# Diamondfan/CTC_pytorch

Measured on AMD Instinct MI355X. Metric: acoustic frames/sec/GPU (train) + utterances/sec beam-decode (`decode` object), TIMIT 4x320 BiLSTM, higher is better.
Workload: dtype f32 via bf16x3 split-operand MFMA (f32 accumulate); 1 GPU; cfg2: 4x320 BiLSTM + BN + Linear(62) + CTC, B=32/GPU, T=800, F=40, dropout 0.1, Adam; global_batch=32, seq_len=800, parallelism=dp1, full_length_utterances=True, sync_bn=False

## Files before the change

ctc_pytorch_amd/_lib.py:

```python
import ctypes
import glob
import os
import subprocess

import torch

_HERE = os.path.dirname(os.path.abspath(__file__))
_CSRC = os.path.join(_HERE, "csrc")
SO_PATH = os.environ.get("CTCN_LIBCTCN") or os.path.join(_HERE, "libctcn.so")
_lib = None

c_void_p, c_int, c_float, c_double, c_size_t, c_u64 = (ctypes.c_void_p, ctypes.c_int, ctypes.c_float,
                                                      ctypes.c_double, ctypes.c_size_t, ctypes.c_uint64)

P, I, F, D, Z, U = c_void_p, c_int, c_float, c_double, c_size_t, c_u64
_SIGS = {
    "ctcn_version": (I, []),
    "ctcn_last_error": (ctypes.c_char_p, []),
    "ctcn_device_cus": (I, []),
    "ctcn_device_xcds": (I, []),
    "ctcn_set_option": (I, [ctypes.c_char_p, I]),
    "ctcn_get_option": (I, [ctypes.c_char_p]),
    "ctcn_option_name": (ctypes.c_char_p, [I]),
    "ctcn_set_status_buffer": (I, [P]),
# ... 23 lines not shown
    "ctcn_bn_bwd_dropout": (I, [P, P, P, P, P, P, P, P, P, I, I, I, I, F, P, Z, P, F, U, U]),
    "ctcn_dropout": (I, [P, P, Z, F, U, U, P]),
    "ctcn_bn_masked_ws_bytes": (Z, [I, I, I]),
    "ctcn_mask_frames": (I, [P, P, P, I, I, I, I, I, P]),
    "ctcn_bn_fwd_train_masked": (I, [P, P, P, P, P, P, P, P, P, I, I, I, I, I, F, F, I, P, Z, P, P]),
    "ctcn_bn_fwd_eval_masked": (I, [P, P, P, P, P, P, P, I, I, I, I, I, F, I, P]),
    "ctcn_bn_bwd_masked": (I, [P, P, P, P, P, P, P, P, P, P, I, I, I, I, I, I, F, P, Z, P]),
    "ctcn_conv2d_ws_bytes": (Z, [I] * 11),
    "ctcn_conv2d_fwd": (I, [P, P, P, P] + [I] * 11 + [P]),
    "ctcn_conv2d_bwd": (I, [P, P, P, P, P, P] + [I] * 11 + [F, P, Z, P]),
    "ctcn_bctf_to_tbcf": (I, [P, P, I, I, I, I, P]),
    "ctcn_tbcf_to_bctf": (I, [P, P, I, I, I, I, P]),
    "ctcn_log_softmax_fwd": (I, [P, P, P, I, I, P]),
    "ctcn_log_softmax_bwd": (I, [P, P, P, I, I, P]),
    "ctcn_argmax": (I, [P, P, I, I, P]),
    "ctcn_rnn_fwd_ex": (I, [I, I, I, I, I, I, P, P, P, P, P, P, P, P, I, P, Z, P, P]),
    "ctcn_rnn_bwd_ex": (I, [I, I, I, I, I, I, P, P, P, P, P, P, P, P, P, P, P, P, P, P, F, I, P, P, Z, P, P]),
    "ctcn_ctc_fwd": (I, [P, P, P, P, P, P, I, I, I, I, P]),
    "ctcn_ctc_bwd": (I, [P, P, P, P, P, P, P, P, I, I, I, I, P]),
    "ctcn_ctc_fwd_both": (I, [P, P, P, P, P, P, P, I, I, I, I, P]),
    "ctcn_ctc_grad": (I, [P, P, P, P, P, P, P, P, P, I, I, I, I, P]),
    "ctcn_sum_f32": (I, [P, P, I, P]),
    "ctcn_ctc_fwd_ex": (I, [P, P, P, P, P, P, P, I, I, I, I, I, P]),
    "ctcn_ctc_grad_ex": (I, [P, P, P, P, P, P, P, P, I, I, I, I, P, I, I, I, I, P]),
    "ctcn_ctc_reduce": (I, [P, P, P, I, I, I, P]),
    "ctcn_ctc_pack_targets": (I, [P, ctypes.c_int64, P, P, I, I, P]),
    "ctcn_ctc_align_ws_bytes": (Z, [I, I, I]),
    "ctcn_ctc_align": (I, [P, P, P, P, P, P, P, P, P, P, I, I, I, I, I, P, Z, P]),
    "ctcn_adam_step": (I, [P, P, P, P, Z, F, F, F, F, F, I, P]),
    "ctcn_grad_norm_ws_bytes": (Z, [Z, I]),
# ... 237 lines not shown
```

ctc_pytorch_amd/csrc/core.hip:

```cpp
#include "common.h"

static thread_local char g_err[512] = "";

void ctcn_set_error(const char *fmt, ...) {
  va_list ap;
  va_start(ap, fmt);
  vsnprintf(g_err, sizeof(g_err), fmt, ap);
  va_end(ap);
}

extern "C" int ctcn_version(void) { return 100; }
extern "C" const char *ctcn_last_error(void) { return g_err; }
extern "C" int ctcn_device_cus(void) {
  int dev = 0, n = 0;
  if (hipGetDevice(&dev) != hipSuccess) return -1;
  if (hipDeviceGetAttribute(&n, hipDeviceAttributeMultiprocessorCount, dev) != hipSuccess) return -1;
  return n;
}

static int g_opt_rnn_persistent = 1;
static int g_opt_handoff = 1;
static int g_opt_poll_depth = 2;
static int g_opt_recurrence_only = 0;
static int g_opt_bwd_scatter = 1;
// ... 18 lines not shown
static int g_opt_gemm_bf16_single = 0;
static int g_opt_gemm_dx_wide = 1;
static int g_opt_xcd_interleave = 1;
static int g_opt_bn_rows4 = 1;
static int g_opt_tn_splits_force = 0;
static int g_opt_tn_splits_xcd = 1;
static int g_opt_beam_generic_threads = 0;
static int g_opt_beam_bitonic = 1;
static int g_opt_beam_cand_global = 0;
static int g_opt_beam_occ2 = 0;
static int g_opt_beam_fast = 1;
static int g_opt_rnn_slow_items = 0;
static int g_opt_rnn_slow_exchange = 0;
static int g_opt_ctc_lattice_skew = 1;
static int g_opt_ctc_slow_wave = 0;
static int g_opt_xcd_interleave_force = 0;
static int *g_status_dev = nullptr;

struct OptionRow { const char *name; int *var; int (*norm)(int); };
static const OptionRow k_options[] = {
  {"rnn_persistent", &g_opt_rnn_persistent, [](int value) -> int { return value; }},
  {"handoff", &g_opt_handoff, [](int value) -> int { return value; }},
  {"poll_depth", &g_opt_poll_depth, [](int value) -> int { return value; }},
  {"rnn_recurrence_only", &g_opt_recurrence_only, [](int value) -> int { return value ? 1 : 0; }},
  {"bwd_scatter", &g_opt_bwd_scatter, [](int value) -> int { return value ? 1 : 0; }},
  {"handoff_tags", &g_opt_handoff_tags, [](int value) -> int { return value ? 1 : 0; }},
  {"side_split_wgs", &g_opt_side_split_wgs, [](int value) -> int { return value < 1 ? 1 : (value > 16 ? 16 : value); }},
  {"gemm_big_tiles", &g_opt_gemm_big_tiles, [](int value) -> int { return value ? 1 : 0; }},
  {"beam_fast", &g_opt_beam_fast, [](int value) -> int { return value ? 1 : 0; }},
  {"conv_dbg", &g_opt_conv_dbg, [](int value) -> int { return value & 7; }},
// ... 13 lines not shown
  {"bwd_item_gather", &g_opt_bwd_item_gather, [](int value) -> int { return value < 0 ? 0 : (value > 2 ? 2 : value); }},
  {"bwd_poll_delay", &g_opt_bwd_poll_delay, [](int value) -> int { return value < 0 ? -1 : (value > 256 ? 256 : value); }},
  {"conv_mfma", &g_opt_conv_mfma, [](int value) -> int { return value ? 1 : 0; }},
  {"edit_wave", &g_opt_edit_wave, [](int value) -> int { return value ? 1 : 0; }},
  {"gemm_tn", &g_opt_gemm_tn, [](int value) -> int { return value != 0; }},
  {"rnn_fused_dropout", &g_opt_rnn_fused_dropout, [](int value) -> int { return value != 0; }},
  {"tag_poll_delay", &g_opt_tag_poll_delay, [](int value) -> int { return value < 0 ? 0 : (value > 64 ? 64 : value); }},
  {"rnn_fwd_tagged", &g_opt_rnn_fwd_tagged, [](int value) -> int { return value ? 1 : 0; }},
  {"gemm_a_inline", &g_opt_gemm_a_inline, [](int value) -> int { return value ? 1 : 0; }},
  {"gemm_dbg", &g_opt_gemm_dbg, [](int value) -> int { return value; }},
  {"gemm_tile256", &g_opt_gemm_tile256, [](int value) -> int { return value ? 1 : 0; }},
  {"xcd_interleave_force", &g_opt_xcd_interleave_force, [](int value) -> int { return value ? 1 : 0; }},
  {"rnn_slow_exchange", &g_opt_rnn_slow_exchange, [](int value) -> int { return value < 0 ? 0 : (value > 4096 ? 4096 : value); }},
  {"ctc_lattice_skew", &g_opt_ctc_lattice_skew, [](int value) -> int { return value ? 1 : 0; }},
  {"ctc_slow_wave", &g_opt_ctc_slow_wave, [](int value) -> int { return value < 0 ? 0 : (value > 15 ? 15 : value); }},
  {"rnn_slow_items", &g_opt_rnn_slow_items, [](int value) -> int { return value < 0 ? 0 : (value > 4096 ? 4096 : value); }},
};
static const int k_noptions = (int)(sizeof(k_options) / sizeof(k_options[0]));
static const OptionRow *find_option(const char *name) {
  if (name)
    for (int i = 0; i < k_noptions; ++i)
      if (!strcmp(name, k_options[i].name)) return &k_options[i];
  return nullptr;
}
extern "C" int ctcn_set_option(const char *name, int value) {
  if (const OptionRow *o = find_option(name)) { *o->var = o->norm(value); return CTCN_OK; }
  ctcn_set_error("ctcn_set_option: unknown option %s", name ? name : "(null)");
  return CTCN_EINVAL;
}
extern "C" int ctcn_get_option(const char *name) {
// ... 15 lines not shown
```

ctc_pytorch_amd/csrc/gemm.hip:

```cpp
#include <algorithm>
#include <type_traits>

#include "common.h"

namespace {

constexpr int BM = 128, BN = 128, BK = 16, PAD = 4;

__device__ __forceinline__ int xcd_band_tile(int bid, int nt) {
  const int xcd = bid & 7, q = nt >> 3, r = nt & 7;
  return (xcd < r ? xcd * (q + 1) : r * (q + 1) + (xcd - r) * q) + (bid >> 3);
}
__device__ __forceinline__ void g2r_kc(const float *__restrict__ src, int ld, int r0, int R, int k0, int Kend,
                                       bool vec, int tid, float (&reg)[8]) {
#pragma unroll
  for (int j = 0; j < 2; ++j) {
    const int idx = tid + 256 * j;
    const int r = idx >> 2, kq = (idx & 3) * 4;
    const int gr = r0 + r, gk = k0 + kq;
    const float *p = src + (size_t)gr * ld + gk;
    if (vec && gr < R && gk + 3 < Kend) {
      const float4 v = *reinterpret_cast<const float4 *>(p);
      reg[4 * j + 0] = v.x; reg[4 * j + 1] = v.y; reg[4 * j + 2] = v.z; reg[4 * j + 3] = v.w;
    } else {
// ... 134 lines not shown
  if (!((xcd_allow >> (x & 15)) & 1u)) return;
  const int nt = tiles_m * tiles_n, total = nt * splits;
  for (;;) {
    if (threadIdx.x == 0) s_item = (int)atomicAdd(queue, 1u);
    __syncthreads();
    const int item = s_item;
    if (item >= total) return;
    f32_tile<TA, TB>(sA, sB, item % nt, item / nt, M, N, K, A, lda, B, ldb, C, ldc, beta, kchunk, ws, tiles_n, vecA, vecB);
    __syncthreads();
  }
}

constexpr int XBK = 32, XLD = 40;
typedef __bf16 bf16x8_t __attribute__((ext_vector_type(8)));

__device__ __forceinline__ void split_bf16(float x, unsigned short &hi, unsigned short &lo) {
  hi = f2bf(x);
  lo = f2bf(x - __uint_as_float((unsigned)hi << 16));
}

__device__ __forceinline__ void x_g2r_kc(const float *__restrict__ src, int ld, int r0, int R, int k0, int Kend, bool vec,
                                         int tid, float (&reg)[16]) {
#pragma unroll
  for (int j = 0; j < 4; ++j) {
    const int idx = tid + 256 * j;
    const int r = idx >> 3, kq = (idx & 7) * 4;
    const int gr = r0 + r, gk = k0 + kq;
    const float *p = src + (size_t)gr * ld + gk;
    if (vec && gr < R && gk + 3 < Kend) {
      const float4 v = *reinterpret_cast<const float4 *>(p);
      reg[4 * j] = v.x; reg[4 * j + 1] = v.y; reg[4 * j + 2] = v.z; reg[4 * j + 3] = v.w;
    } else {
#pragma unroll
      for (int c = 0; c < 4; ++c) reg[4 * j + c] = (gr < R && gk + c < Kend) ? p[c] : 0.0f;
// ... 1753 lines not shown
```

ctc_pytorch_amd/csrc/norm.hip:

```cpp
#include <algorithm>

#include "common.h"

namespace {

struct Pair { double a, b; };

struct StatVal {
  const float *x;
  __device__ __forceinline__ Pair operator()(size_t idx, int) const {
    const double v = x[idx];
    return {v, v * v};
  }
  struct Quad { f32x4 x; };
  __device__ __forceinline__ Quad load4(size_t idx) const { return {*reinterpret_cast<const f32x4 *>(x + idx)}; }
  __device__ __forceinline__ void add4(const Quad &q, int, double &a, double &b) const {
#pragma unroll
    for (int e = 0; e < 4; ++e) { const double v = q.x[e]; a += v; b += v * v; }
  }
  __host__ __device__ __forceinline__ bool aligned16() const { return ((uintptr_t)x & 15) == 0; }
  struct ColK {};
  static constexpr int ROWS_IN_FLIGHT = 8;
  __device__ __forceinline__ ColK colk(int) const { return {}; }
  __device__ __forceinline__ void cols4(const Quad &q, const ColK &, double (&a)[4], double (&b)[4]) const {
#pragma unroll
    for (int e = 0; e < 4; ++e) { const double v = q.x[e]; a[e] += v; b[e] += v * v; }
  }
};
struct DropSpec { float p, scale; uint64_t seed, offset; const float *gamma, *beta; };
__device__ __forceinline__ float bn_value(float x, float m, float rs, float g, float b) { return fmaf((x - m) * rs, g, b); }
__device__ __forceinline__ bool drop_keep(uint32_t word, float p) { return (word >> 8) * (1.0f / 16777216.0f) >= p; }
__device__ __forceinline__ float bn_dx_value(float g, float xh, float ga, float rs, float s0, float s1, float inv_n) {
  return ga * rs * fmaf(-xh, s1 * inv_n, fmaf(-s0, inv_n, g));
}

struct BwdVal {
  const float *x, *y, *dy, *mean, *rstd;
  int relu;
  DropSpec d;
  __device__ __forceinline__ Pair operator()(size_t idx, int c) const {
    float g = dy[idx];
    if (d.p > 0.0f) {
      uint32_t r[4];
      philox4(d.seed, d.offset + (idx >> 2), r);
      g = drop_keep(r[idx & 3], d.p) ? g * d.scale : 0.0f;
      if (relu && !(bn_value(x[idx], mean[c], rstd[c], d.gamma[c], d.beta[c]) > 0.0f)) g = 0.0f;
    } else if (relu && !(y[idx] > 0.0f)) g = 0.0f;
    const float xh = (x[idx] - mean[c]) * rstd[c];
    return {(double)g, (double)g * (double)xh};
// ... 599 lines not shown
  return ws_part_bytes(outer, C, inner) + (size_t)2 * C * sizeof(float);
}

extern "C" size_t ctcn_bn_masked_ws_bytes(int outer, int C, int inner) {
  const size_t n = ctcn_bn_ws_bytes(outer, C, inner);
  return n ? n + 256 : 0;
}

extern "C" int ctcn_bn_fwd_train(const float *x, float *y, const float *gamma, const float *beta, float *running_mean,
                                 float *running_var, float *save_mean, float *save_rstd, int outer, int C, int inner,
                                 float eps, float momentum, int relu, void *ws, size_t ws_bytes, void *stream, long long *num_batches_tracked) {
  return bn_forward("ctcn_bn_fwd_train", all_frames((double)outer * inner), dims_ok(outer, C, inner), x, y, gamma, beta, running_mean, running_var,
                    save_mean, save_rstd, outer, C, inner, eps, momentum, relu, ws, ws_bytes, stream, num_batches_tracked, nullptr);
}

extern "C" int ctcn_bn_fwd_train_dropout(const float *x, float *y_drop, const float *gamma, const float *beta, float *running_mean, float *running_var,
                                         float *save_mean, float *save_rstd, int outer, int C, int inner, float eps, float momentum, int relu, void *ws,
                                         size_t ws_bytes, void *stream, long long *num_batches_tracked, float p, uint64_t seed, uint64_t offset) {
  const DropSpec d = drop_spec(p, seed, offset, gamma, beta);
  return bn_forward("ctcn_bn_fwd_train_dropout", all_frames((double)outer * inner), dims_ok(outer, C, inner), x, y_drop, gamma, beta, running_mean,
                    running_var, save_mean, save_rstd, outer, C, inner, eps, momentum, relu, ws, ws_bytes, stream, num_batches_tracked, &d);
}

extern "C" int ctcn_bn_fwd_train_masked(const float *x, float *y, const float *gamma, const float *beta, float *running_mean, float *running_var,
                                        float *save_mean, float *save_rstd, const int *lens, int batch, int frame, int outer, int C, int inner,
                                        float eps, float momentum, int relu, void *ws, size_t ws_bytes, void *stream, long long *num_batches_tracked) {
  Frames g = {};
  const bool geom = geom_ok(outer, C, inner, lens, batch, frame, &g);
  return bn_forward("ctcn_bn_fwd_train_masked", g, geom, x, y, gamma, beta, running_mean, running_var, save_mean, save_rstd, outer, C, inner, eps,
                    momentum, relu, ws, ws_bytes, stream, num_batches_tracked, nullptr);
// ... 118 lines not shown
```

ctc_pytorch_amd/models/model_ctc.py:

```python
import math
import os
import sys
from collections import OrderedDict

import numpy as np
import torch

_ROOT = os.path.dirname(os.path.dirname(os.path.dirname(os.path.abspath(__file__))))
if _ROOT not in sys.path:
    sys.path.insert(0, _ROOT)

from ctc_pytorch_amd import nn, ops

F = nn.functional

__author__ = "ctc_pytorch_amd (MI355X-native rebuild; class surface after Ruchao Fan's CTC_pytorch)"


class BatchRNN(nn.Module):

    def __init__(self, input_size, hidden_size, rnn_type=nn.LSTM, bidirectional=False, batch_norm=True, dropout=0.1):
        super().__init__()
        self.input_size = input_size
        self.hidden_size = hidden_size
# ... 193 lines not shown
            h = ops.contiguous(h.transpose(0, 1))
        for n, block in enumerate(self.rnns):
            h = block(h, lengths=None if n == 0 and block.batch_norm is None else lens)
        Tp = h.shape[0]
        h = h.reshape(Tp * B, -1)
        if isinstance(self.fc, nn.Sequential):
            z = self.fc[1](self.fc[0](h, lengths=lens))
        else:
            z = self.fc(ops.mask_frames(h.view(Tp, B, -1), lens, "tbc").view(Tp * B, -1))
        out = self.log_softmax(z.view(Tp, B, -1))
        if visualize:
            visual.append(out)
            return out, visual
        return out

    def forward(self, x, visualize=False, input_lengths=None):
        if input_lengths is not None:
            return self._forward_masked(x, visualize, input_lengths)
        visual = [x] if visualize else None
        if self.add_cnn:
            c = self.conv(x.unsqueeze(1))
            if visualize:
                visual.append(c)
            if c.dim() != 4:
                raise NotImplementedError("Conv1d front-end")
            h = ops.bctf_to_tbcf(c)
            if visualize:
                visual.append(h)
        else:
            h = ops.contiguous(x.transpose(0, 1))
        h = self.rnns(h)
        T, B, _ = h.shape
        z = self.fc(h.reshape(T * B, -1))
        out = self.log_softmax(z.view(T, B, -1))
        if visualize:
            visual.append(out)
            return out, visual
        return out

    def compute_wer(self, index, input_sizes, targets, target_sizes):
        dev = next(self.parameters()).device
        idx = torch.as_tensor(np.asarray(index) if not torch.is_tensor(index) else index).to(dev).to(torch.int32)
        lens = torch.as_tensor(np.asarray(input_sizes) if not torch.is_tensor(input_sizes) else input_sizes).to(dev)
        tg = torch.as_tensor(np.asarray(targets) if not torch.is_tensor(targets) else targets).to(dev)
        tl = torch.as_tensor(np.asarray(target_sizes) if not torch.is_tensor(target_sizes) else target_sizes).to(dev)
        ids, ids_len = ops.greedy_collapse(idx, lens, blank=0, batch_major=True)
        dist = ops.edit_distance(ids, ids_len, tg, tl)
        return int(dist.sum().item()), int(tl.sum().item())

# ... 24 lines not shown
```

ctc_pytorch_amd/ops.py:

```python
import collections
import ctypes
import os
import numpy as np

import torch

from . import _lib

CELL = {"lstm": 0, "gru": 1, "tanh": 2}
GATES = {0: 4, 1: 3, 2: 1}

def _precision_from_env():
    v = os.environ.get("CTCN_PRECISION", "1").strip()
    if v not in ("0", "1"):
        raise ValueError("CTCN_PRECISION must be 0 (exact f32 MFMA) or 1 (bf16x3 split-operand MFMA), got %r" % v)
    return int(v)


DEFAULT_PRECISION = _precision_from_env()
_precision = [DEFAULT_PRECISION]


def set_precision(p):
    if int(p) not in (0, 1):
# ... 1021 lines not shown

    @staticmethod
    def backward(ctx, g):
        (lp,) = ctx.saved_tensors
        g = _f32c(g)
        V = lp.shape[-1]
        dz = torch.empty_like(lp)
        _lib.check(_lib.lib().ctcn_log_softmax_bwd(_ptr(lp), _ptr(g), _ptr(dz), lp.numel() // V, V, _lib.stream_ptr()), "log_softmax_bwd")
        return dz


def log_softmax(z):
    return _LogSoftmax.apply(z)


def argmax_last(lp):
    _need_gpu(lp)
    lp = _f32c(lp.detach())
    V = lp.shape[-1]
    out = torch.empty(lp.shape[:-1], dtype=torch.int32, device=lp.device)
    _lib.check(_lib.lib().ctcn_argmax(_ptr(lp), _ptr(out), lp.numel() // V, V, _lib.stream_ptr()), "argmax")
    return out


_REDUCTIONS = {"none": 0, "mean": 1, "sum": 2}

CtcArgs = collections.namedtuple("CtcArgs", "lp targets in_len tgt_len Lmax flat batched")


def _lengths(x):
# ... 1118 lines not shown
```

include/ctcn.h:

```cpp
#ifndef CTCN_H
#define CTCN_H
#include <stddef.h>
#include <stdint.h>
#ifdef __cplusplus
extern "C" {
#endif

#define CTCN_OK 0
#define CTCN_EINVAL (-1)
#define CTCN_EHIP (-2)
#define CTCN_EUNSUPPORTED (-3)
#define CTCN_EWORKSPACE (-4)

#define CTCN_REDUCTION_NONE 0
#define CTCN_REDUCTION_MEAN 1
#define CTCN_REDUCTION_SUM 2

#define CTCN_CELL_LSTM 0
#define CTCN_CELL_GRU 1
#define CTCN_CELL_TANH 2

int ctcn_version(void);
const char *ctcn_last_error(void);
int ctcn_device_cus(void);
// ... 99 lines not shown

int ctcn_dropout(const float *x, float *y, size_t n, float p, uint64_t seed, uint64_t offset, void *stream);

size_t ctcn_conv2d_ws_bytes(int B, int Ci, int Hi, int Wi, int Co, int kh, int kw, int sh, int sw, int ph, int pw);
int ctcn_conv2d_fwd(const float *x, const float *w, const float *bias, float *y, int B, int Ci, int Hi, int Wi,
                    int Co, int kh, int kw, int sh, int sw, int ph, int pw, void *stream);
int ctcn_conv2d_bwd(const float *x, const float *w, const float *dy, float *dx , float *dw,
                    float *dbias, int B, int Ci, int Hi, int Wi, int Co, int kh, int kw, int sh, int sw, int ph,
                    int pw, float beta_acc, void *ws, size_t ws_bytes, void *stream);
int ctcn_bctf_to_tbcf(const float *in, float *out, int B, int C, int T, int F, void *stream);
int ctcn_tbcf_to_bctf(const float *in, float *out, int B, int C, int T, int F, void *stream);

int ctcn_log_softmax_fwd(const float *logits, float *lp, int32_t *argmax, int rows, int V, void *stream);
int ctcn_log_softmax_bwd(const float *lp, const float *dlp, float *dlogits, int rows, int V, void *stream);
int ctcn_argmax(const float *lp, int32_t *argmax, int rows, int V, void *stream);

int ctcn_ctc_fwd(const float *lp, const int64_t *targets, const int64_t *in_len, const int64_t *tgt_len,
                 float *alpha, float *nll, int T, int B, int V, int Lmax, void *stream);
int ctcn_ctc_bwd(const float *lp, const int64_t *targets, const int64_t *in_len, const int64_t *tgt_len,
                 float *alpha, const float *nll, const float *gscale, float *grad_lp, int T, int B, int V,
                 int Lmax, void *stream);
int ctcn_ctc_fwd_both(const float *lp, const int64_t *targets, const int64_t *in_len, const int64_t *tgt_len,
                      float *alpha, float *beta, float *nll, int T, int B, int V, int Lmax, void *stream);
int ctcn_ctc_grad(const float *lp, const int64_t *targets, const int64_t *in_len, const int64_t *tgt_len,
                  const float *alpha, const float *beta, const float *nll, const float *gscale, float *grad_lp,
                  int T, int B, int V, int Lmax, void *stream);
int ctcn_sum_f32(const float *x, float *out, int n, void *stream);
int ctcn_ctc_fwd_ex(const float *lp, const int64_t *targets, const int64_t *in_len, const int64_t *tgt_len, float *alpha,
                    float *beta, float *nll, int T, int B, int V, int Lmax, int blank, void *stream);
int ctcn_ctc_grad_ex(const float *lp, const int64_t *targets, const int64_t *in_len, const int64_t *tgt_len, const float *alpha,
// ... 188 lines not shown
```

Baseline: 2.009 million frames/s.

## Fuse BatchNorm, Linear and LogSoftmax head into dedicated forward/backward kernels

Adds a fused output head that applies the BatchNorm normalisation on the fly while staging the GEMM operand, runs the Linear via bf16x3 MFMA, and computes log-softmax in the epilogue, so the normalised activations and the logits are never written to memory. The backward pass is also fused: log-softmax backward, the dW/dgamma/dbeta partial sums, a finalize reduction and the dx computation with the BN gradient. It is meant to cut the memory traffic and kernel launches of the separate BN, GEMM and softmax ops at the top of the model. In exchange it adds a large amount of new kernel code, per-tile partial buffers, and an eligibility check that falls back to the old path.

Result: no change. 2.016 million frames/s, median of 6 (+0.3%).

```diff
diff --git a/ctc_pytorch_amd/_lib.py b/ctc_pytorch_amd/_lib.py
--- a/ctc_pytorch_amd/_lib.py
+++ b/ctc_pytorch_amd/_lib.py
@@ -61,6 +61,13 @@
     "ctcn_log_softmax_fwd": (I, [P, P, P, I, I, P]),
     "ctcn_log_softmax_bwd": (I, [P, P, P, I, I, P]),
     "ctcn_argmax": (I, [P, P, I, I, P]),
+    "ctcn_diag_head_plan": (I, [I, I, I, I, ctypes.c_uint, P]),
+    "ctcn_head_ws_bytes": (Z, [I, I, I]),
+    "ctcn_bn_fwd_stats": (I, [P, P, P, P, P, I, I, I, F, F, P, Z, P, P]),
+    "ctcn_head_fwd": (I, [P, P, P, P, P, P, P, I, I, I, I, P]),
+    "ctcn_head_bwd_sums": (I, [P, P, P, P, P, P, P, P, I, I, I, I, P, Z, P]),
+    "ctcn_head_bwd_finalize": (I, [P, P, P, I, I, I, I, I, P, Z, P]),
+    "ctcn_head_bwd_dx": (I, [P, P, P, P, P, P, P, P, I, I, I, I, P, Z, P]),
     "ctcn_rnn_fwd_ex": (I, [I, I, I, I, I, I, P, P, P, P, P, P, P, P, I, P, Z, P, P]),
     "ctcn_rnn_bwd_ex": (I, [I, I, I, I, I, I, P, P, P, P, P, P, P, P, P, P, P, P, P, P, F, I, P, P, Z, P, P]),
     "ctcn_ctc_fwd": (I, [P, P, P, P, P, P, I, I, I, I, P]),
diff --git a/ctc_pytorch_amd/csrc/core.hip b/ctc_pytorch_amd/csrc/core.hip
--- a/ctc_pytorch_amd/csrc/core.hip
+++ b/ctc_pytorch_amd/csrc/core.hip
@@ -56,6 +56,7 @@
 static int g_opt_rnn_slow_exchange = 0;
 static int g_opt_ctc_lattice_skew = 1;
 static int g_opt_ctc_slow_wave = 0;
+static int g_opt_head_fused = 1;
 static int g_opt_xcd_interleave_force = 0;
 static int *g_status_dev = nullptr;
 
@@ -99,6 +100,7 @@
   {"rnn_slow_exchange", &g_opt_rnn_slow_exchange, [](int value) -> int { return value < 0 ? 0 : (value > 4096 ? 4096 : value); }},
   {"ctc_lattice_skew", &g_opt_ctc_lattice_skew, [](int value) -> int { return value ? 1 : 0; }},
   {"ctc_slow_wave", &g_opt_ctc_slow_wave, [](int value) -> int { return value < 0 ? 0 : (value > 15 ? 15 : value); }},
+  {"head_fused", &g_opt_head_fused, [](int value) -> int { return value < 0 ? 0 : (value > 2 ? 2 : value); }},
   {"rnn_slow_items", &g_opt_rnn_slow_items, [](int value) -> int { return value < 0 ? 0 : (value > 4096 ? 4096 : value); }},
 };
 static const int k_noptions = (int)(sizeof(k_options) / sizeof(k_options[0]));
diff --git a/ctc_pytorch_amd/csrc/device_math.h b/ctc_pytorch_amd/csrc/device_math.h
--- /dev/null
+++ b/ctc_pytorch_amd/csrc/device_math.h
@@ -0,0 +1,27 @@
+#pragma once
+#include "common.h"
+
+__device__ __forceinline__ void split_bf16(float x, unsigned short &hi, unsigned short &lo) {
+  hi = f2bf(x);
+  lo = f2bf(x - __uint_as_float((unsigned)hi << 16));
+}
+
+__device__ __forceinline__ float bn_value(float x, float m, float rs, float g, float b) { return fmaf((x - m) * rs, g, b); }
+__device__ __forceinline__ float bn_dx_value(float g, float xh, float ga, float rs, float s0, float s1, float inv_n) {
+  return ga * rs * fmaf(-xh, s1 * inv_n, fmaf(-s0, inv_n, g));
+}
+
+__device__ __forceinline__ float log_softmax_lane(float x, bool on) {
+  const float m = wave_max(on ? fmaxf(-INFINITY, x) : -INFINITY);
+  float s = 0.0f;
+  if (on) s += expf(x - m);
+  s = wave_sum(s);
+  const float lse = m + logf(s);
+  return x - lse;
+}
+__device__ __forceinline__ float log_softmax_bwd_lane(float lp, float g, bool on) {
+  float s = 0.0f;
+  if (on) s += g;
+  s = wave_sum(s);
+  return on ? g - expf(lp) * s : 0.0f;
+}
diff --git a/ctc_pytorch_amd/csrc/gemm.hip b/ctc_pytorch_amd/csrc/gemm.hip
--- a/ctc_pytorch_amd/csrc/gemm.hip
+++ b/ctc_pytorch_amd/csrc/gemm.hip
@@ -2,6 +2,7 @@
 #include <type_traits>
 
 #include "common.h"
+#include "device_math.h"
 
 namespace {
 
@@ -172,10 +173,6 @@
 constexpr int XBK = 32, XLD = 40;
 typedef __bf16 bf16x8_t __attribute__((ext_vector_type(8)));
 
-__device__ __forceinline__ void split_bf16(float x, unsigned short &hi, unsigned short &lo) {
-  hi = f2bf(x);
-  lo = f2bf(x - __uint_as_float((unsigned)hi << 16));
-}
 
 __device__ __forceinline__ void x_g2r_kc(const float *__restrict__ src, int ld, int r0, int R, int k0, int Kend, bool vec,
                                          int tid, float (&reg)[16]) {
diff --git a/ctc_pytorch_amd/csrc/head.hip b/ctc_pytorch_amd/csrc/head.hip
--- /dev/null
+++ b/ctc_pytorch_amd/csrc/head.hip
@@ -0,0 +1,394 @@
+#include <algorithm>
+
+#include "common.h"
+#include "device_math.h"
+
+namespace {
+
+constexpr int HR = 128;
+constexpr int HK = 64;
+constexpr int HLD = HK + 8;
+constexpr int HLT = HR + 8;
+constexpr int HV = 64;
+typedef __bf16 bf16x8_t __attribute__((ext_vector_type(8)));
+typedef unsigned short (*img_k)[HLD];
+typedef unsigned short (*img_r)[HLT];
+
+__device__ __forceinline__ int acc_row(int e, int lane) { return (e & 3) + 8 * (e >> 2) + 4 * (lane >> 5); }
+
+__device__ __forceinline__ void mfma_x3(f32x16 &acc, bf16x8_t ah, bf16x8_t al, bf16x8_t bh, bf16x8_t bl) {
+  acc = __builtin_amdgcn_mfma_f32_32x32x16_bf16(al, bh, acc, 0, 0, 0);
+  acc = __builtin_amdgcn_mfma_f32_32x32x16_bf16(ah, bl, acc, 0, 0, 0);
+  acc = __builtin_amdgcn_mfma_f32_32x32x16_bf16(ah, bh, acc, 0, 0, 0);
+}
+template <int LD>
+__device__ __forceinline__ bf16x8_t frag(const unsigned short (*img)[LD], int row, int k) { return *reinterpret_cast<const bf16x8_t *>(&img[row][k]); }
+
+__device__ __forceinline__ void store_split4(unsigned short *hi, unsigned short *lo, const float (&v)[4]) {
+  unsigned short h[4], l[4];
+#pragma unroll
+  for (int e = 0; e < 4; ++e) split_bf16(v[e], h[e], l[e]);
+  *reinterpret_cast<uint2 *>(hi) = make_uint2((unsigned)h[0] | ((unsigned)h[1] << 16), (unsigned)h[2] | ((unsigned)h[3] << 16));
+  *reinterpret_cast<uint2 *>(lo) = make_uint2((unsigned)l[0] | ((unsigned)l[1] << 16), (unsigned)l[2] | ((unsigned)l[3] << 16));
+}
+
+__device__ __forceinline__ f32x4 load_w4(const float *p, bool vec) {
+  if (vec) return *reinterpret_cast<const f32x4 *>(p);
+  return f32x4{p[0], p[1], p[2], p[3]};
+}
+
+__global__ __launch_bounds__(256) void head_fwd_kernel(const float *__restrict__ h, const float *__restrict__ mean, const float *__restrict__ rstd,
+                                                       const float *__restrict__ gamma, const float *__restrict__ beta, const float *__restrict__ W,
+                                                       float *__restrict__ lp, int R, int C, int V, bool wvec) {
+  __shared__ __attribute__((aligned(16))) unsigned char sm[(2 * HR + 2 * HV) * HLD * 2];
+  img_k sAh = (img_k)sm, sAl = sAh + HR, sBh = sAl + HR, sBl = sBh + HV;
+  float(*sZ)[HV + 1] = (float(*)[HV + 1])sm;
+  static_assert(sizeof(float) * HR * (HV + 1) <= sizeof(sm), "the logits tile lies over the staging images");
+  const int tid = threadIdx.x, lane = tid & 63, wave = tid >> 6;
+  const int r0 = blockIdx.x * HR;
+  const int kq = (tid & 15) * 4, rr = tid >> 4;
+
+  f32x16 acc[2];
+#pragma unroll
+  for (int j = 0; j < 2; ++j)
+#pragma unroll
+    for (int e = 0; e < 16; ++e) acc[j][e] = 0.0f;
+
+  f32x4 ra0[8], ra1[8], ra2[8], rb[4], m, rs, ga, be;
+  auto aload = [&](int k0, f32x4 (&ra)[8]) {
+    const int kc = k0 + kq < C ? k0 + kq : 0;
+#pragma unroll
+    for (int j = 0; j < 8; ++j) ra[j] = *reinterpret_cast<const f32x4 *>(h + (size_t)min(r0 + rr + 16 * j, R - 1) * C + kc);
+  };
+  auto wload = [&](int k0) {
+    const int kc = k0 + kq < C ? k0 + kq : 0;
+#pragma unroll
+    for (int e = 0; e < 4; ++e) {
+      m[e] = mean[kc + e]; rs[e] = rstd[kc + e]; ga[e] = gamma[kc + e]; be[e] = beta[kc + e];
+    }
+#pragma unroll
+    for (int j = 0; j < 4; ++j) rb[j] = load_w4(W + (size_t)min(rr + 16 * j, V - 1) * C + kc, wvec);
+  };
+  auto stage = [&](int k0, f32x4 (&ra)[8]) {
+    const bool kin = k0 + kq < C;
+    lds_barrier();
+#pragma unroll
+    for (int j = 0; j < 8; ++j) {
+      const bool in = kin && r0 + rr + 16 * j < R;
+      float v[4];
+#pragma unroll
+      for (int e = 0; e < 4; ++e) v[e] = in ? bn_value(ra[j][e], m[e], rs[e], ga[e], be[e]) : 0.0f;
+      store_split4(&sAh[rr + 16 * j][kq], &sAl[rr + 16 * j][kq], v);
+    }
+#pragma unroll
+    for (int j = 0; j < 4; ++j) {
+      const bool in = kin && rr + 16 * j < V;
+      const float v[4] = {in ? rb[j][0] : 0.0f, in ? rb[j][1] : 0.0f, in ? rb[j][2] : 0.0f, in ? rb[j][3] : 0.0f};
+      store_split4(&sBh[rr + 16 * j][kq], &sBl[rr + 16 * j][kq], v);
+    }
+    lds_barrier();
+    if (k0 + HK < C) wload(k0 + HK);
+    if (k0 + 3 * HK < C) aload(k0 + 3 * HK, ra);
+    const int ml = lane & 31, kg = (lane >> 5) * 8;
+#pragma unroll
+    for (int ks = 0; ks < HK; ks += 16) {
+      const bf16x8_t ah = frag(sAh, wave * 32 + ml, ks + kg), al = frag(sAl, wave * 32 + ml, ks + kg);
+#pragma unroll
+      for (int j = 0; j < 2; ++j) mfma_x3(acc[j], ah, al, frag(sBh, j * 32 + ml, ks + kg), frag(sBl, j * 32 + ml, ks + kg));
+    }
+  };
+  wload(0);
+  aload(0, ra0);
+  if (HK < C) aload(HK, ra1);
+  if (2 * HK < C) aload(2 * HK, ra2);
+  for (int k0 = 0; k0 < C; k0 += 3 * HK) {
+    stage(k0, ra0);
+    if (k0 + HK < C) stage(k0 + HK, ra1);
+    if (k0 + 2 * HK < C) stage(k0 + 2 * HK, ra2);
+  }
+  __syncthreads();
+#pragma unroll
+  for (int j = 0; j < 2; ++j)
+#pragma unroll
+    for (int e = 0; e < 16; ++e) sZ[wave * 32 + acc_row(e, lane)][j * 32 + (lane & 31)] = acc[j][e];
+  __syncthreads();
+  for (int i = wave; i < HR && r0 + i < R; i += 4) {
+    const bool on = lane < V;
+    const float v = log_softmax_lane(on ? sZ[i][lane] : 0.0f, on);
+    if (on) lp[(size_t)(r0 + i) * V + lane] = v;
+  }
+}
+
+struct HeadBwdLds {
+  static constexpr int dzA = 0, wT = dzA + 2 * HR * HLD * 2, end_dx = wT + 2 * HK * HLD * 2;
+  static constexpr int dzT = end_dx, xT = dzT + 2 * HV * HLT * 2, red = xT + 2 * HK * HLT * 2, end_sums = red + 2 * 8 * HK * 8;
+};
+
+struct HeadChunk {
+  float h[2][16];
+  f32x4 w[4];
+  float m[2], rs[2], ga[2], be[2], s0[2], s1[2];
+};
+
+template <bool DX>
+__global__ __launch_bounds__(256) void head_bwd_kernel(const float *__restrict__ G, const float *__restrict__ lp, const float *__restrict__ h,
+                                                       const float *__restrict__ mean, const float *__restrict__ rstd, const float *__restrict__ gamma,
+                                                       const float *__restrict__ beta, const float *__restrict__ W, int R, int C, int V,
+                                                       double *__restrict__ part_bn, float *__restrict__ part_dw, const float *__restrict__ sums,
+                                                       float inv_n, float *__restrict__ dh, bool wvec) {
+  extern __shared__ __attribute__((aligned(16))) unsigned char hsm[];
+  img_k dzAh = (img_k)(hsm + HeadBwdLds::dzA), dzAl = dzAh + HR, sWh = (img_k)(hsm + HeadBwdLds::wT), sWl = sWh + HK;
+  img_r dzTh = (img_r)(hsm + HeadBwdLds::dzT), dzTl = dzTh + HV, sXh = (img_r)(hsm + HeadBwdLds::xT), sXl = sXh + HK;
+  double(*red)[8][HK] = (double(*)[8][HK])(hsm + HeadBwdLds::red);
+  const int tid = threadIdx.x, lane = tid & 63, wave = tid >> 6;
+  const int ml = lane & 31, g = lane >> 5, kg = g * 8;
+  const int r0 = blockIdx.x * HR;
+  const int kq = (tid & 15) * 4, rr = tid >> 4;
+
+  auto fetch = [&](int c0, HeadChunk &k) {
+#pragma unroll
+    for (int j = 0; j < 2; ++j) {
+      const int c = min(c0 + 32 * j + ml, C - 1);
+      k.m[j] = mean[c]; k.rs[j] = rstd[c]; k.ga[j] = gamma[c];
+      if (DX) { k.s0[j] = sums[c]; k.s1[j] = sums[C + c]; }
+      else k.be[j] = beta[c];
+#pragma unroll
+      for (int e = 0; e < 16; ++e) k.h[j][e] = h[(size_t)min(r0 + 32 * wave + acc_row(e, lane), R - 1) * C + c];
+    }
+    const int kc = c0 + kq < C ? c0 + kq : 0;
+#pragma unroll
+    for (int j = 0; j < 4; ++j) k.w[j] = load_w4(W + (size_t)min(rr + 16 * j, V - 1) * C + kc, wvec);
+  };
+  HeadChunk ka, kb, kc;
+  fetch(0, ka);
+  if (HK < C) fetch(HK, kb);
+  if (2 * HK < C) fetch(2 * HK, kc);
+
+  for (int i = wave; i < HR; i += 4) {
+    const int row = r0 + i;
+    float dz = 0.0f;
+    if (row < R) {
+      const bool on = lane < V;
+      dz = log_softmax_bwd_lane(on ? lp[(size_t)row * V + lane] : 0.0f, on ? G[(size_t)row * V + lane] : 0.0f, on);
+    }
+    unsigned short hi, lo;
+    split_bf16(dz, hi, lo);
+    dzAh[i][lane] = hi; dzAl[i][lane] = lo;
+    if (!DX) { dzTh[lane][i] = hi; dzTl[lane][i] = lo; }
+  }
+
+  auto chunk = [&](int c0, HeadChunk &k) {
+#pragma unroll
+    for (int j = 0; j < 4; ++j) {
+      const int v = rr + 16 * j;
+      const bool in = v < V && c0 + kq < C;
+#pragma unroll
+      for (int e = 0; e < 4; ++e) {
+        unsigned short hi, lo;
+        split_bf16(in ? k.w[j][e] : 0.0f, hi, lo);
+        sWh[kq + e][v] = hi; sWl[kq + e][v] = lo;
+      }
+    }
+    if (!DX) {
+#pragma unroll
+      for (int j = 0; j < 2; ++j) {
+        const bool cin = c0 + 32 * j + ml < C;
+#pragma unroll
+        for (int q = 0; q < 4; ++q) {
+          float v[4];
+#pragma unroll
+          for (int e = 0; e < 4; ++e) {
+            const bool in = cin && r0 + 32 * wave + 8 * q + 4 * g + e < R;
+            v[e] = in ? bn_value(k.h[j][4 * q + e], k.m[j], k.rs[j], k.ga[j], k.be[j]) : 0.0f;
+          }
+          store_split4(&sXh[32 * j + ml][32 * wave + 8 * q + 4 * g], &sXl[32 * j + ml][32 * wave + 8 * q + 4 * g], v);
+        }
+      }
+    }
+    lds_barrier();
+
+    f32x16 gx[2];
+#pragma unroll
+    for (int j = 0; j < 2; ++j)
+#pragma unroll
+      for (int e = 0; e < 16; ++e) gx[j][e] = 0.0f;
+#pragma unroll
+    for (int ks = 0; ks < HV; ks += 16) {
+      const bf16x8_t ah = frag(dzAh, wave * 32 + ml, ks + kg), al = frag(dzAl, wave * 32 + ml, ks + kg);
+#pragma unroll
+      for (int j = 0; j < 2; ++j) mfma_x3(gx[j], ah, al, frag(sWh, j * 32 + ml, ks + kg), frag(sWl, j * 32 + ml, ks + kg));
+    }
+
+    if (DX) {
+#pragma unroll
+      for (int j = 0; j < 2; ++j) {
+        const int c = c0 + 32 * j + ml;
+        if (c < C) {
+#pragma unroll
+          for (int e = 0; e < 16; ++e) {
+            const int row = r0 + 32 * wave + acc_row(e, lane);
+            const float xh = (k.h[j][e] - k.m[j]) * k.rs[j];
+            if (row < R) dh[(size_t)row * C + c] = bn_dx_value(gx[j][e], xh, k.ga[j], k.rs[j], k.s0[j], k.s1[j], inv_n);
+          }
+        }
+      }
+    } else {
+#pragma unroll
+      for (int j = 0; j < 2; ++j) {
+        double a = 0.0, b = 0.0;
+#pragma unroll
+        for (int e = 0; e < 16; ++e) {
+          const float xh = (k.h[j][e] - k.m[j]) * k.rs[j];
+          a += (double)gx[j][e]; b += (double)gx[j][e] * (double)xh;
+        }
+        red[0][2 * wave + g][32 * j + ml] = a; red[1][2 * wave + g][32 * j + ml] = b;
+      }
+      const int vt = wave & 1, ct = wave >> 1;
+      f32x16 dw;
+#pragma unroll
+      for (int e = 0; e < 16; ++e) dw[e] = 0.0f;
+#pragma unroll
+      for (int ks = 0; ks < HR; ks += 16)
+        mfma_x3(dw, frag(dzTh, vt * 32 + ml, ks + kg), frag(dzTl, vt * 32 + ml, ks + kg), frag(sXh, ct * 32 + ml, ks + kg), frag(sXl, ct * 32 + ml, ks + kg));
+      const int c = c0 + 32 * ct + ml;
+      if (c < C) {
+#pragma unroll
+        for (int e = 0; e < 16; ++e) {
+          const int v = 32 * vt + acc_row(e, lane);
+          if (v < V) part_dw[((size_t)blockIdx.x * V + v) * C + c] = dw[e];
+        }
+      }
+    }
+    if (c0 + 3 * HK < C) fetch(c0 + 3 * HK, k);
+    lds_barrier();
+    if (!DX && tid < HK && c0 + tid < C) {
+      double a = red[0][0][tid], b = red[1][0][tid];
+#pragma unroll
+      for (int q = 1; q < 8; ++q) { a += red[0][q][tid]; b += red[1][q][tid]; }
+      part_bn[((size_t)blockIdx.x * C + c0 + tid) * 2 + 0] = a;
+      part_bn[((size_t)blockIdx.x * C + c0 + tid) * 2 + 1] = b;
+    }
+  };
+  for (int c0 = 0; c0 < C; c0 += 3 * HK) {
+    chunk(c0, ka);
+    if (c0 + HK < C) chunk(c0 + HK, kb);
+    if (c0 + 2 * HK < C) chunk(c0 + 2 * HK, kc);
+  }
+}
+
+__global__ __launch_bounds__(256) void head_finalize_kernel(const double *__restrict__ part_bn, const float *__restrict__ part_dw, int tiles, int C, int V,
+                                                            float *__restrict__ sums, float *__restrict__ dgamma, float *__restrict__ dbeta,
+                                                            float *__restrict__ dW, int bn_acc, int w_acc) {
+  __shared__ double sa[8][32], sb[8][32];
+  const int el = threadIdx.x & 31, grp = threadIdx.x >> 5;
+  const size_t i = (size_t)blockIdx.x * 32 + el, nw = (size_t)V * C;
+  const int per = (tiles + 7) / 8, k0 = grp * per, k1 = min(tiles, k0 + per);
+  double a = 0.0, b = 0.0;
+  if (i < nw) {
+    int k = k0;
+    for (; k + 8 <= k1; k += 8) {
+      float v[8];
+#pragma unroll
+      for (int u = 0; u < 8; ++u) v[u] = part_dw[(size_t)(k + u) * nw + i];
+#pragma unroll
+      for (int u = 0; u < 8; ++u) a += (double)v[u];
+    }
+    for (; k < k1; ++k) a += (double)part_dw[(size_t)k * nw + i];
+  } else if (i < nw + C) {
+    const size_t c = i - nw;
+    for (int k = k0; k < k1; ++k) { a += part_bn[((size_t)k * C + c) * 2]; b += part_bn[((size_t)k * C + c) * 2 + 1]; }
+  }
+  sa[grp][el] = a; sb[grp][el] = b;
+  __syncthreads();
+  if (grp != 0 || i >= nw + C) return;
+  for (int q = 1; q < 8; ++q) { a += sa[q][el]; b += sb[q][el]; }
+  if (i < nw) {
+    dW[i] = (float)a + (w_acc ? dW[i] : 0.0f);
+  } else {
+    const size_t c = i - nw;
+    sums[c] = (float)a; sums[C + c] = (float)b;
+    dbeta[c] = (float)a + (bn_acc ? dbeta[c] : 0.0f);
+    dgamma[c] = (float)b + (bn_acc ? dgamma[c] : 0.0f);
+  }
+}
+
+struct HeadPlan { bool eligible; int tiles; size_t off_dw, off_sums, bytes; };
+constexpr int HEAD_MIN_TILES = 128;
+HeadPlan plan_head(int rows, int C, int V, int precision, unsigned align_or) {
+  HeadPlan p = {};
+  if (rows <= 0 || C <= 0 || V <= 0) return p;
+  p.tiles = ceil_div(rows, HR);
+  p.off_dw = align_up((size_t)p.tiles * C * 2 * sizeof(double), 256);
+  p.off_sums = p.off_dw + align_up((size_t)p.tiles * V * C * sizeof(float), 256);
+  p.bytes = p.off_sums + (size_t)2 * C * sizeof(float);
+  const int opt = ctcn_get_option("head_fused");
+  p.eligible = precision == 1 && V <= HV && C <= 960 && C % 4 == 0 && (align_or & 15u) == 0 && ctcn_get_option("gemm_bf16_single") == 0 &&
+               (opt == 2 || (opt == 1 && p.tiles >= HEAD_MIN_TILES));
+  return p;
+}
+
+}
+
+extern "C" int ctcn_diag_head_plan(int rows, int C, int V, int precision, unsigned align_or, int *out) {
+  CTCN_REQUIRE(out && rows > 0 && C > 0 && V > 0, "ctcn_diag_head_plan: bad args");
+  const HeadPlan p = plan_head(rows, C, V, precision, align_or);
+  const int v[CTCN_HEAD_PLAN_INTS] = {p.eligible, p.tiles, (int)(HeadBwdLds::end_sums), (int)(HeadBwdLds::end_dx)};
+  memcpy(out, v, sizeof(v));
+  return CTCN_OK;
+}
+
+extern "C" size_t ctcn_head_ws_bytes(int rows, int C, int V) { return plan_head(rows, C, V, 1, 0u).bytes; }
+
+#define HEAD_ELIGIBLE(who, p)                                                                                                   \
+  CTCN_REQUIRE((p).eligible, "%s: rows=%d C=%d V=%d precision=%d is outside the fused head (ctcn_diag_head_plan); take the unfused path", who, rows, C, V, \
+               precision)
+
+extern "C" int ctcn_head_fwd(const float *h, const float *mean, const float *rstd, const float *gamma, const float *beta, const float *W, float *lp,
+                             int rows, int C, int V, int precision, void *stream) {
+  CTCN_REQUIRE(h && mean && rstd && gamma && beta && W && lp && rows > 0 && C > 0 && V > 0, "ctcn_head_fwd: bad args");
+  const HeadPlan p = plan_head(rows, C, V, precision, (unsigned)(uintptr_t)h);
+  HEAD_ELIGIBLE("ctcn_head_fwd", p);
+  hipLaunchKernelGGL(head_fwd_kernel, dim3(p.tiles), dim3(256), 0, (hipStream_t)stream, h, mean, rstd, gamma, beta, W, lp, rows, C, V, ((uintptr_t)W & 15) == 0);
+  CTCN_LAUNCH_CHECK();
+  return CTCN_OK;
+}
+
+extern "C" int ctcn_head_bwd_sums(const float *g, const float *lp, const float *h, const float *mean, const float *rstd, const float *gamma,
+                                  const float *beta, const float *W, int rows, int C, int V, int precision, void *ws, size_t ws_bytes, void *stream) {
+  CTCN_REQUIRE(g && lp && h && mean && rstd && gamma && beta && W && ws && rows > 0 && C > 0 && V > 0, "ctcn_head_bwd_sums: bad args");
+  CTCN_REQUIRE((uintptr_t)ws % 16 == 0, "ctcn_head_bwd_sums: the workspace must be 16-byte aligned");
+  const HeadPlan p = plan_head(rows, C, V, precision, (unsigned)(uintptr_t)h);
+  HEAD_ELIGIBLE("ctcn_head_bwd_sums", p);
+  if (ws_bytes < p.bytes) { ctcn_set_error("ctcn_head_bwd_sums: workspace too small"); return CTCN_EWORKSPACE; }
+  auto kern = head_bwd_kernel<false>;
+  CTCN_HIP(hipFuncSetAttribute(reinterpret_cast<const void *>(kern), hipFuncAttributeMaxDynamicSharedMemorySize, HeadBwdLds::end_sums));
+  hipLaunchKernelGGL(kern, dim3(p.tiles), dim3(256), HeadBwdLds::end_sums, (hipStream_t)stream, g, lp, h, mean, rstd, gamma, beta, W, rows, C, V,
+                     (double *)ws, (float *)((char *)ws + p.off_dw), (const float *)nullptr, 0.0f, (float *)nullptr, ((uintptr_t)W & 15) == 0);
+  CTCN_LAUNCH_CHECK();
+  return CTCN_OK;
+}
+
+extern "C" int ctcn_head_bwd_finalize(float *dgamma, float *dbeta, float *dW, int rows, int C, int V, int bn_acc, int w_acc, void *ws, size_t ws_bytes,
+                                      void *stream) {
+  CTCN_REQUIRE(dgamma && dbeta && dW && ws && rows > 0 && C > 0 && V > 0, "ctcn_head_bwd_finalize: bad args");
+  const HeadPlan p = plan_head(rows, C, V, 1, 0u);
+  if (ws_bytes < p.bytes) { ctcn_set_error("ctcn_head_bwd_finalize: workspace too small"); return CTCN_EWORKSPACE; }
+  const size_t n = (size_t)V * C + C;
+  hipLaunchKernelGGL(head_finalize_kernel, dim3((unsigned)ceil_div_z(n, 32)), dim3(256), 0, (hipStream_t)stream, (const double *)ws,
+                     (const float *)((char *)ws + p.off_dw), p.tiles, C, V, (float *)((char *)ws + p.off_sums), dgamma, dbeta, dW, bn_acc, w_acc);
+  CTCN_LAUNCH_CHECK();
+  return CTCN_OK;
+}
+
+extern "C" int ctcn_head_bwd_dx(const float *g, const float *lp, const float *h, const float *mean, const float *rstd, const float *gamma,
+                                const float *W, float *dh, int rows, int C, int V, int precision, void *ws, size_t ws_bytes, void *stream) {
+  CTCN_REQUIRE(g && lp && h && mean && rstd && gamma && W && dh && ws && rows > 0 && C > 0 && V > 0, "ctcn_head_bwd_dx: bad args");
+  const HeadPlan p = plan_head(rows, C, V, precision, (unsigned)((uintptr_t)h | (uintptr_t)dh));
+  HEAD_ELIGIBLE("ctcn_head_bwd_dx", p);
+  if (ws_bytes < p.bytes) { ctcn_set_error("ctcn_head_bwd_dx: workspace too small"); return CTCN_EWORKSPACE; }
+  auto kern = head_bwd_kernel<true>;
+  hipLaunchKernelGGL(kern, dim3(p.tiles), dim3(256), HeadBwdLds::end_dx, (hipStream_t)stream, g, lp, h, mean, rstd, gamma, gamma, W, rows, C, V,
+                     (double *)nullptr, (float *)nullptr, (const float *)((char *)ws + p.off_sums), (float)(1.0 / (double)rows), dh, ((uintptr_t)W & 15) == 0);
+  CTCN_LAUNCH_CHECK();
+  return CTCN_OK;
+}
diff --git a/ctc_pytorch_amd/csrc/norm.hip b/ctc_pytorch_amd/csrc/norm.hip
--- a/ctc_pytorch_amd/csrc/norm.hip
+++ b/ctc_pytorch_amd/csrc/norm.hip
@@ -1,6 +1,7 @@
 #include <algorithm>
 
 #include "common.h"
+#include "device_math.h"
 
 namespace {
 
@@ -28,11 +29,7 @@
   }
 };
 struct DropSpec { float p, scale; uint64_t seed, offset; const float *gamma, *beta; };
-__device__ __forceinline__ float bn_value(float x, float m, float rs, float g, float b) { return fmaf((x - m) * rs, g, b); }
 __device__ __forceinline__ bool drop_keep(uint32_t word, float p) { return (word >> 8) * (1.0f / 16777216.0f) >= p; }
-__device__ __forceinline__ float bn_dx_value(float g, float xh, float ga, float rs, float s0, float s1, float inv_n) {
-  return ga * rs * fmaf(-xh, s1 * inv_n, fmaf(-s0, inv_n, g));
-}
 
 struct BwdVal {
   const float *x, *y, *dy, *mean, *rstd;
@@ -662,6 +659,22 @@
                     save_mean, save_rstd, outer, C, inner, eps, momentum, relu, ws, ws_bytes, stream, num_batches_tracked, nullptr);
 }
 
+extern "C" int ctcn_bn_fwd_stats(const float *x, float *running_mean, float *running_var, float *save_mean, float *save_rstd, int outer, int C, int inner,
+                                 float eps, float momentum, void *ws, size_t ws_bytes, void *stream, long long *num_batches_tracked) {
+  CTCN_REQUIRE(x && save_mean && save_rstd && ws, "ctcn_bn_fwd_stats: null pointer");
+  CTCN_REQUIRE(dims_ok(outer, C, inner), "ctcn_bn_fwd_stats: bad dims");
+  if (ws_bytes < ctcn_bn_ws_bytes(outer, C, inner)) { ctcn_set_error("ctcn_bn_fwd_stats: workspace too small"); return CTCN_EWORKSPACE; }
+  hipStream_t st = (hipStream_t)stream;
+  const AllFrames g = all_frames((double)outer * inner);
+  int nchunks = 0;
+  launch_reduce(StatVal{x}, g, outer, C, inner, (double *)ws, &nchunks, st);
+  CTCN_LAUNCH_CHECK();
+  hipLaunchKernelGGL(bn_finalize_stats_kernel<AllFrames>, dim3(ceil_div(C, 4)), dim3(256), 0, st, (const double *)ws, nchunks, C, g, eps, momentum, save_mean,
+                     save_rstd, running_mean, running_var, num_batches_tracked);
+  CTCN_LAUNCH_CHECK();
+  return CTCN_OK;
+}
+
 extern "C" int ctcn_bn_fwd_train_dropout(const float *x, float *y_drop, const float *gamma, const float *beta, float *running_mean, float *running_var,
                                          float *save_mean, float *save_rstd, int outer, int C, int inner, float eps, float momentum, int relu, void *ws,
                                          size_t ws_bytes, void *stream, long long *num_batches_tracked, float p, uint64_t seed, uint64_t offset) {
diff --git a/ctc_pytorch_amd/models/model_ctc.py b/ctc_pytorch_amd/models/model_ctc.py
--- a/ctc_pytorch_amd/models/model_ctc.py
+++ b/ctc_pytorch_amd/models/model_ctc.py
@@ -231,6 +231,13 @@
             return out, visual
         return out
 
+    def _head_modules(self):
+        fc = self.fc
+        if isinstance(fc, nn.Sequential) and len(fc) == 2 and type(fc[0]) is nn.BatchNorm1d and type(fc[1]) is nn.Linear and fc[1].bias is None \
+                and type(self.log_softmax) is nn.LogSoftmax and self.log_softmax.dim in (-1, 2):
+            return fc[0], fc[1]
+        return None
+
     def forward(self, x, visualize=False, input_lengths=None):
         if input_lengths is not None:
             return self._forward_masked(x, visualize, input_lengths)
@@ -248,8 +255,11 @@
             h = ops.contiguous(x.transpose(0, 1))
         h = self.rnns(h)
         T, B, _ = h.shape
-        z = self.fc(h.reshape(T * B, -1))
-        out = self.log_softmax(z.view(T, B, -1))
+        h = h.reshape(T * B, -1)
+        if self._head_modules() is not None and ops.head_fused_eligible(h, *self._head_modules()):
+            out = ops.head_fused(h, *self._head_modules()).view(T, B, -1)
+        else:
+            out = self.log_softmax(self.fc(h).view(T, B, -1))
         if visualize:
             visual.append(out)
             return out, visual
diff --git a/ctc_pytorch_amd/ops.py b/ctc_pytorch_amd/ops.py
--- a/ctc_pytorch_amd/ops.py
+++ b/ctc_pytorch_amd/ops.py
@@ -1059,6 +1059,81 @@
     return _LogSoftmax.apply(z)
 
 
+def head_plan(rows, C, V, align_or=0, precision=None):
+    out = (ctypes.c_int * 4)()
+    prec = get_precision() if precision is None else int(precision)
+    _lib.check(_lib.lib().ctcn_diag_head_plan(int(rows), int(C), int(V), prec, int(align_or) & 0xffffffff, ctypes.cast(out, ctypes.c_void_p)), "diag_head_plan")
+    return dict(zip(("fused", "tiles", "lds_sums", "lds_dx"), (int(v) for v in out)))
+
+
+def head_fused_eligible(h, bn, lin, lengths=None):
+    if lengths is not None or _sync_bn["reduce"] is not None or not (bn.training and bn.affine and bn.track_running_stats) or bn.fuse_relu:
+        return False
+    if lin.bias is not None or h.dim() != 2 or not h.is_cuda or h.dtype != torch.float32 or not h.is_contiguous() or h.shape[0] < 1:
+        return False
+    if h.shape[1] != bn.num_features or lin.weight.shape[1] != h.shape[1] or not lin.weight.is_contiguous():
+        return False
+    return bool(head_plan(h.shape[0], h.shape[1], lin.weight.shape[0], h.data_ptr())["fused"])
+
+
+class _HeadFused(torch.autograd.Function):
+
+    @staticmethod
+    def forward(ctx, h, gamma, beta, w, rm, rv, nbt, momentum, eps):
+        _need_gpu(h, gamma, beta, w)
+        ctx.gviews = (_gview(gamma), _gview(beta), _gview(w))
+        rows, C = h.shape
+        V = w.shape[0]
+        dev = h.device
+        L = _lib.lib()
+        mean = torch.empty(C, dtype=torch.float32, device=dev)
+        rstd = torch.empty(C, dtype=torch.float32, device=dev)
+        lp = torch.empty((rows, V), dtype=torch.float32, device=dev)
+        ws, wp, wn = _ws(h)
+        _lib.check(L.ctcn_bn_fwd_stats(_ptr(h), _ptr(rm), _ptr(rv), _ptr(mean), _ptr(rstd), rows, C, 1, float(eps), float(momentum), wp, wn,
+                                       _lib.stream_ptr(), _ptr(nbt)), "bn_fwd_stats")
+        ctx.prec = get_precision()
+        _lib.check(L.ctcn_head_fwd(_ptr(h), _ptr(mean), _ptr(rstd), _ptr(gamma), _ptr(beta), _ptr(w), _ptr(lp), rows, C, V, ctx.prec,
+                                   _lib.stream_ptr()), "head_fwd")
+        ctx.save_for_backward(h, gamma, beta, w, mean, rstd, lp)
+        return lp
+
+    @staticmethod
+    def backward(ctx, g):
+        h, gamma, beta, w, mean, rstd, lp = ctx.saved_tensors
+        g = _f32c(g)
+        rows, C = h.shape
+        V = w.shape[0]
+        dev = h.device
+        L = _lib.lib()
+        st = _lib.stream_ptr()
+        ws, wp, wn = _ws(h)
+        gv_g, gv_b, gv_w = ctx.gviews
+        bn_flat = gv_g is not None and gv_b is not None
+        dgamma, dbeta = (gv_g, gv_b) if bn_flat else (torch.empty(C, dtype=torch.float32, device=dev), torch.empty(C, dtype=torch.float32, device=dev))
+        dw = gv_w if gv_w is not None else torch.empty((V, C), dtype=torch.float32, device=dev)
+        dh = torch.empty_like(h)
+        if not head_plan(rows, C, V, h.data_ptr() | dh.data_ptr(), ctx.prec)["fused"]:
+            raise RuntimeError("ctc_pytorch_amd: the fused head's backward no longer covers the call its forward took (option or precision changed in between)")
+        _lib.check(L.ctcn_head_bwd_sums(_ptr(g), _ptr(lp), _ptr(h), _ptr(mean), _ptr(rstd), _ptr(gamma), _ptr(beta), _ptr(w), rows, C, V, ctx.prec,
+                                        wp, wn, st), "head_bwd_sums")
+        _lib.check(L.ctcn_head_bwd_finalize(_ptr(dgamma), _ptr(dbeta), _ptr(dw), rows, C, V, int(bn_flat), int(gv_w is not None), wp, wn, st),
+                   "head_bwd_finalize")
+        _lib.check(L.ctcn_head_bwd_dx(_ptr(g), _ptr(lp), _ptr(h), _ptr(mean), _ptr(rstd), _ptr(gamma), _ptr(w), _ptr(dh), rows, C, V, ctx.prec,
+                                      wp, wn, st), "head_bwd_dx")
+        return (dh if ctx.needs_input_grad[0] else None, None if bn_flat else dgamma, None if bn_flat else dbeta, None if gv_w is not None else dw,
+                None, None, None, None, None)
+
+
+def head_fused(h, bn, lin):
+    nbt = bn.num_batches_tracked
+    if nbt is not None and (nbt.dtype != torch.int64 or not nbt.is_cuda):
+        nbt += 1
+        nbt = None
+    mom = 0.1 if bn.momentum is None else bn.momentum
+    return _HeadFused.apply(h, bn.weight, bn.bias, lin.weight, bn.running_mean, bn.running_var, nbt, mom, bn.eps)
+
+
 def argmax_last(lp):
     _need_gpu(lp)
     lp = _f32c(lp.detach())
diff --git a/include/ctcn.h b/include/ctcn.h
--- a/include/ctcn.h
+++ b/include/ctcn.h
@@ -137,6 +137,20 @@
 int ctcn_log_softmax_fwd(const float *logits, float *lp, int32_t *argmax, int rows, int V, void *stream);
 int ctcn_log_softmax_bwd(const float *lp, const float *dlp, float *dlogits, int rows, int V, void *stream);
 int ctcn_argmax(const float *lp, int32_t *argmax, int rows, int V, void *stream);
+
+#define CTCN_HEAD_PLAN_INTS 4
+int ctcn_diag_head_plan(int rows, int C, int V, int precision, unsigned align_or, int *out);
+size_t ctcn_head_ws_bytes(int rows, int C, int V);
+int ctcn_bn_fwd_stats(const float *x, float *running_mean, float *running_var, float *save_mean, float *save_rstd, int outer, int C, int inner,
+                      float eps, float momentum, void *ws, size_t ws_bytes, void *stream, long long *num_batches_tracked);
+int ctcn_head_fwd(const float *h, const float *mean, const float *rstd, const float *gamma, const float *beta, const float *W, float *lp,
+                  int rows, int C, int V, int precision, void *stream);
+int ctcn_head_bwd_sums(const float *g, const float *lp, const float *h, const float *mean, const float *rstd, const float *gamma,
+                       const float *beta, const float *W, int rows, int C, int V, int precision, void *ws, size_t ws_bytes, void *stream);
+int ctcn_head_bwd_finalize(float *dgamma, float *dbeta, float *dW, int rows, int C, int V, int bn_acc, int w_acc, void *ws, size_t ws_bytes,
+                           void *stream);
+int ctcn_head_bwd_dx(const float *g, const float *lp, const float *h, const float *mean, const float *rstd, const float *gamma,
+                     const float *W, float *dh, int rows, int C, int V, int precision, void *ws, size_t ws_bytes, void *stream);
 
 int ctcn_ctc_fwd(const float *lp, const int64_t *targets, const int64_t *in_len, const int64_t *tgt_len,
                  float *alpha, float *nll, int T, int B, int V, int Lmax, void *stream);
```
